# ACCtools/alignasm

Measured on AMD Instinct MI355X. Metric: contigs_per_sec, higher is better.
Workload: dtype int64

## Files before the change

alignasm_amd/csrc/aasm_kernels.h:

```cpp
#pragma once
#include <cstddef>
#include "aasm_dev.h"
#include "../../include/alignasm_amd.h"

namespace aasm {

struct PqK;
struct WS {
    int64_t C, R, R0, S, VT, ET;
    int32_t K, nsl;
    int32_t avg_sidetracks;
    int32_t xcd_map;
    int32_t mw_compact;
    int32_t sort_depth_test;
    const int64_t *rec_off, *in_qs, *in_qe, *in_rs, *in_re, *in_qt, *in_rng_off, *rql, *rqr, *rrl;
    const int32_t *in_chr;
    const uint8_t *in_fwd, *in_mq;
    const char *cs_text;
    const int64_t *cs_off;
    int64_t *rng_rec;
    int64_t rng_stride;
    int32_t *cs_bad;
    int32_t *perm, *dupflag, *np, *pstart;
    int64_t *s_qs, *s_qe, *s_rs, *s_re, *s_qt, *s_rb;
    int32_t *s_rn, *s_chr, *s_orig, *s_ctg, *s_pid;
    uint8_t *s_fl;
    int32_t *ov_cnt, *ov_rec, *ov_vid;
    int64_t *ov_off, *ov_rank, *ov_peq, *ov_per, *ov_stq, *ov_str;
    uint8_t *ov_ok;
    int32_t *dis_end, *next_cnt;
    int32_t *ctgV, *v_i, *v_j, *v_ctg;
    int64_t *voff, *v_slot;
    int32_t *deg, *e_col, *e_wr, *indeg, *rcur, *r_e;
    I4 *tmp_pk;
    int64_t *rowptr, *e_wq, *rptr;
    uint8_t *e_fl;
    Dist *sp_d;
    int32_t *sp_best, *rev_order, *cnt_tmp, *fwd_order, *fwd_pos, *an, *anom_dest, *cnt_tmp2;
    int32_t *tp_deg, *tp_vj;
    int64_t *tp_ptr;
    I4 *te_pk;
    int32_t *ccnt, *cval;
    int64_t *hoff;
    int32_t *hcap_cnt;
    HNode *hnodes;
    int32_t *h_root, *bq, *h_cnt;
    Dist *kd;
    int32_t *klast, *kfound;
    I4 *kcand;
    PqK *pq;
    int64_t pq_stride;
    int32_t *pathA, *pathB, *pathT, *pre2, *stamp;
    Dist *dist2;
    uint8_t *notalt;
    int32_t *mark_time;
    int32_t *plan_kk;
    int32_t *nconv, *cv_ctg, *cv_k, *cv_ord, *cv_kind, *cv_szr, *cv_szv, *cv_n, *cv_err, *cv_path, *cv_pre2, *cv_stamp, *cv_la;
    int64_t *conv_off, *cv_roff, *cv_voff, *cv_cov;
    OutElem *cv_out;
    Dist *cv_dist2;
    int64_t NCONV;
    OutElem *cur_out, *main_out, *alt_out, *pool;
    int32_t *main_len, *alt_len, *all_gen, *all_seq;
    int32_t *ar_ctg, *ar_gen, *ar_seq, *ar_len;
    int64_t *ar_off;
    int64_t pool_cap, ar_cap;
    int64_t *main_off, *alt_off;
    OutElem *main_c, *alt_c;
    int32_t *status;
    int64_t *counters;
    int32_t *gb_flag; int32_t gb_off;
    int64_t *prof_heap, *prof_sel, *prof_gb;
    Dist *st_cost;
    int32_t *st_n;
    I4 *vhdr, *vhdr2, *cinfo;
    int32_t mw_mode;
    int32_t *mw_flag, *mw_lg;
    HNode *hprov;
    int64_t *mw_off;
    int32_t *mw_cap;
    int32_t *mw_order, *mw_rs, *mw_fb;
    int32_t *mw_rsv, *mw_used;
    int32_t *mw_list, *mw_sorted;
    int32_t *mw_key;
    int32_t mw_n, mw_base;
    I4 *tnx;
    int32_t *tnx16;
    I4 *rvh;
    I4 *r_pk;
    I4 *fvh;
    int32_t chain_mode;
    int32_t chain_all, chain_minN;
    int32_t chain_test;
    int32_t *chain_flag, *chain_list;
    int32_t *pend;
    int32_t *cq;
    I4 *bfsq;
    int32_t chain_ord;
    int32_t chain_rn;
};

enum { CNT_RANGE_STEPS = 0, CNT_UNCONN, CNT_POOL, CNT_AR, CNT_CONVERTED, CNT_HEAPNODES, CNT_PATHS, CNT_OVF, CNT_ISPR_E, CNT_ISPR_V, CNT_PATH_E, CNT_OUT_E, CNT_PQ_PUSH, CNT_MW, CNT_MAXN, CNT_LONGSORT, CNT_MAXV, CNT_CHAIN, CNT_GB_S, CNT_GB_L, CNT_GB_REST, CNT_N };

AASM_DEV void set_status(const WS &w, int64_t c, int code) { if (w.status[c] == 0) w.status[c] = code; }
AASM_DEV bool in_chain_class(const WS &w, int64_t c) { return w.chain_flag != nullptr && w.chain_flag[c] != 0; }
AASM_DEV bool in_graph_class(const WS &w, int64_t c) { return w.gb_flag && w.gb_flag[c] != 0; }
#define AASM_COORD_LIMIT ((int64_t)1 << 40)
AASM_DEV bool coord_ok(int64_t x) { return x >= 0 && x < AASM_COORD_LIMIT; }

AASM_DEV bool cs_is_op(int c) { return c == ':' || c == '*' || c == '+' || c == '-'; }
struct CsScan {
    int64_t q, rr, val, n, cnt, o0;
    int32_t plen;
    int t;
    bool fwd, bad;
};
AASM_DEV void cs_close_op(CsScan &s, const WS &w) {
    if (s.t == ':') {
        if (s.plen < 1 || s.val <= 0 || s.n >= s.cnt) { s.bad = true; return; }
        if (s.fwd) {
            const int64_t o = s.o0 + s.n;
            I4 lo, hi; const int64_t qr = s.q + s.val - 1;
            lo.x = lo32((uint64_t)s.q); lo.y = hi32((uint64_t)s.q); lo.z = lo32((uint64_t)qr); lo.w = hi32((uint64_t)qr);
            hi.x = lo32((uint64_t)s.rr); hi.y = hi32((uint64_t)s.rr); hi.z = 0; hi.w = 0;
            I4 *rec = (I4 *)(w.rng_rec + 4 * o); rec[0] = lo; rec[1] = hi;
            s.q += s.val;
        } else {
            const int64_t o = s.o0 + s.cnt - 1 - s.n;
            I4 lo, hi; const int64_t ql = s.q - s.val, qr = s.q - 1, rl = s.rr + s.val - 1;
            lo.x = lo32((uint64_t)ql); lo.y = hi32((uint64_t)ql); lo.z = lo32((uint64_t)qr); lo.w = hi32((uint64_t)qr);
            hi.x = lo32((uint64_t)rl); hi.y = hi32((uint64_t)rl); hi.z = 0; hi.w = 0;
            I4 *rec = (I4 *)(w.rng_rec + 4 * o); rec[0] = lo; rec[1] = hi;
            s.q -= s.val;
        }
        s.rr += s.val;
        s.n++;
    } else if (s.t == '*') {
        if (s.plen != 2) { s.bad = true; return; }
        s.q += s.fwd ? 1 : -1; s.rr += 1;
    } else {
        if (s.plen < 1) { s.bad = true; return; }
        if (s.t == '+') s.q += s.fwd ? s.plen : -s.plen; else s.rr += s.plen;
    }
}
AASM_DEV void kb_cs_ranges(const KCtx &k, const WS &w) {
    const int64_t br = k.bid * k.nthreads + k.tid;
    if (br >= w.R) return;
    const int64_t r = w.R0 + br;
    const int64_t p0 = w.cs_off[r], len = w.cs_off[r + 1] - p0;
    const uint8_t *cs = (const uint8_t *)w.cs_text + p0;
    const int64_t qs = w.in_qs[r], qe = w.in_qe[r], rs = w.in_rs[r], re = w.in_re[r];
    CsScan s;
    s.fwd = w.in_fwd[r] != 0;
    s.o0 = w.in_rng_off[r]; s.cnt = w.in_rng_off[r + 1] - s.o0;
    s.q = s.fwd ? qs : qe + 1; s.rr = s.fwd ? rs : re;
// ... 1818 lines not shown
    if (gv >= w.VT || in_chain_class(w, w.v_ctg[gv]) || in_graph_class(w, w.v_ctg[gv])) return;
    tnx16_vertex(w, gv);
}
#define TNX_TPB 256
#define AASM_TNXWG_LDS_BYTES (GB_MAXV_L * 4)
AASM_DEV void kb_tnx16_wg(const KCtx &k, const WS &w) {
    const int64_t c = k.bid;
    const int64_t V = w.ctgV[c];
    if (V == 0 || !in_graph_class(w, c) || in_chain_class(w, c)) return;
    int32_t *Lb = (int32_t *)k.lds;
    const int64_t vb = w.voff[c];
    for (int32_t v = k.tid; v < V; v += k.nthreads) Lb[v] = w.sp_best[vb + v];
    block_barrier();
    for (int32_t v = k.tid; v < V; v += k.nthreads) {
        I4 *o = (I4 *)(w.tnx16 + 16 * (vb + v));
        int32_t x = v;
        AASM_UNROLL
        for (int t = 0; t < 4; t++) {
            I4 j;
            x = x >= 0 ? Lb[x] : -1; j.x = x;
            x = x >= 0 ? Lb[x] : -1; j.y = x;
            x = x >= 0 ? Lb[x] : -1; j.z = x;
            x = x >= 0 ? Lb[x] : -1; j.w = x;
            o[t] = j;
        }
    }
}
AASM_DEV void kb_k7_prep(const KCtx &k, const WS &w) {
    const int64_t gv = k.bid * k.nthreads + k.tid;
    if (gv >= w.VT || in_chain_class(w, w.v_ctg[gv])) return;
    int32_t ch4[4];
    const int32_t nch = children_vertex(w, gv, ch4);
    const int32_t nkeys = sidetrack_vertex(w, gv);
    I4 a, b;
    heap_hdr_vertex(w, gv, a, b, nch, ch4, nkeys);
    w.vhdr[gv] = a; w.vhdr2[gv] = b;
}
AASM_DEV void kb_heap_hdr(const KCtx &k, const WS &w) {
    const int64_t gv = k.bid * k.nthreads + k.tid;
    if (gv >= w.VT || in_chain_class(w, w.v_ctg[gv])) return;
    I4 a, b;
    heap_hdr_vertex(w, gv, a, b);
    w.vhdr[gv] = a; w.vhdr2[gv] = b;
}

AASM_DEV void kb_heap_cap(const KCtx &k, const WS &w) {
    const int64_t c = k.bid * k.nthreads + k.tid;
    if (c >= w.C) return;
    const int64_t V = w.ctgV[c];
    w.mw_flag[c] = 0; w.mw_cap[c] = 0; w.mw_lg[c] = 2;
    if (w.chain_flag) w.chain_flag[c] = 0;
    w.gb_flag[c] = 0;
    if (V == 0) { w.hcap_cnt[c] = 0; return; }
    const int64_t vb = w.voff[c];
    const int64_t E = w.rowptr[vb + V] - w.rowptr[vb];
    {
        const bool sparse_batch = w.rowptr[w.VT] <= 6 * w.VT;
        const int32_t f = (w.gb_off || !sparse_batch) ? 0 : (V <= GB_MAXV && E <= GB_MAXE) ? 1 : (V <= GB_MAXV_L && E <= GB_MAXE_L) ? 2 : 0;
        w.gb_flag[c] = f;
        atomic_add(&w.counters[f == 1 ? CNT_GB_S : f == 2 ? CNT_GB_L : CNT_GB_REST], (int64_t)1);
    }
    if (E > (int64_t)INT32_MAX - 64) { w.status[c] = -5; w.hcap_cnt[c] = 0; return; }
    int64_t I = E - (V - 1);
    if (I < 0) I = 0;
    int lg = 0;
    for (int64_t t = I + 1; t > 1; t >>= 1) lg++;
    int64_t cap = I * (lg + 2) + 8;
    if (cap > 0x7fffff00) cap = 0x7fffff00;
    w.mw_lg[c] = lg + 2;
    w.mw_flag[c] = (w.mw_mode == 1 || (w.mw_mode == 0 && I >= 6 * V && V >= 128)) ? 1 : 0;
    w.mw_cap[c] = w.mw_flag[c] ? (int32_t)cap : 0;
    w.hcap_cnt[c] = (w.mw_flag[c] && !w.mw_compact) ? 0 : (int32_t)cap;
    if (w.mw_flag[c]) { const int64_t slot = atomic_add(&w.counters[CNT_MW], (int64_t)1); w.mw_list[slot] = (int32_t)c; w.mw_key[slot] = (int32_t)cap; }
    if (w.chain_flag) {
        const int64_t N = w.rec_off[c + 1] - w.rec_off[c];
        const bool sparse_batch = w.rowptr[w.VT] <= 6 * w.VT;
        const bool in = !w.mw_flag[c] && sparse_batch && w.status[c] == 0 &&
                        (w.chain_mode == 1 || (w.chain_mode == 0 && (w.chain_all || (w.chain_minN > 0 && N >= w.chain_minN))));
        w.chain_flag[c] = in ? 1 : 0;
        if (in) { const int64_t slot = atomic_add(&w.counters[CNT_CHAIN], (int64_t)1); w.chain_list[slot] = (int32_t)c; }
    }
}

#define HEAP_RING 64
#define HEAP_QN 128
#define HEAP_KMAX 16
struct HeapStage { Dist key[HEAP_KMAX]; };
#define HEAP_OLDN 8
template <int RING, int QN> struct HeapLdsT {
    HNode ring[RING];
    I4 bq[QN];
    HeapStage stage;
    HNode bounce;
    HNode oldn[HEAP_OLDN];
};
#define HEAP_RING_1W 64
#define HEAP_QN_1W 128
#define HEAP_RING_CH 256
#define HEAP_QN_CH 128
#define AASM_HEAP_LDS_BYTES_T(RING, QN) ((RING) * 48 + (QN) * 16 + HEAP_KMAX * 32 + 48 + HEAP_OLDN * 48)
#define AASM_HEAP_LDS_BYTES AASM_HEAP_LDS_BYTES_T(HEAP_RING_1W, HEAP_QN_1W)
static_assert(sizeof(HeapLdsT<HEAP_RING_1W, HEAP_QN_1W>) <= AASM_HEAP_LDS_BYTES && sizeof(HeapLdsT<HEAP_RING_CH, HEAP_QN_CH>) <= AASM_HEAP_LDS_BYTES_T(HEAP_RING_CH, HEAP_QN_CH), "LDS budget");
struct Spine {
    LaneArr<NodeQ> n;
    LaneArr<int32_t> idx;
    LaneArr<int64_t> sum;
    LaneArr<int32_t> t;
    int32_t root, len, tail;
};
struct HeapState {
    HNode *nodes;
    HNode *ring;
    int32_t rn;
    HNode *bounce;
    HNode *oldn;
    int32_t alloc, flushed, cap;
    int32_t ring_lo;
    bool ovf;
};

AASM_DEV const HNode *heap_arena(const WS &w, int64_t c) { return (w.mw_flag[c] && !w.mw_compact) ? w.hprov + w.mw_off[c] : w.hnodes + w.hoff[c]; }
AASM_DEV NodeQ heap_read(const HeapState &hs, int32_t a, HNode *slot = nullptr) {
    NodeQ n;
    const HNode *src = &hs.ring[a & (hs.rn - 1)];
    if (!slot) slot = hs.bounce;
    if (!(a >= hs.alloc - hs.rn && a >= hs.ring_lo)) {
        const NodeQ g = nodeq_load(&hs.nodes[a]);
        asm volatile("" ::: "memory");
        nodeq_store(slot, g);
        src = slot;
    }
    n = nodeq_load(src);
    return n;
}
AASM_DEV bool nodeq_key_lt(const NodeQ &n, const Dist &key, int64_t ksum) {
    const Dist nk = nodeq_key(n);
    const int64_t nsum = nk.qry + nk.ref;
    if (nsum != ksum && nsum != -2 && ksum != -2) return nsum < ksum;
    return dist_lt<CALC_SUM_MODE>(nk, key);
}
AASM_DEV bool key_tie_lt(const NodeQ &n, const Dist &key) {
    const int32_t na = n.q1.x, nn = n.q1.y, nt = n.q1.z ? n.q1.z : 1, kt = key.qtot ? key.qtot : 1;
    return (na < key.anom) | ((na == key.anom) & ((int64_t)nn * (int64_t)kt > (int64_t)key.qnz * (int64_t)nt));
}
AASM_DEV void heap_flush(HeapState &hs, int lane) {
    const int32_t m = hs.alloc - hs.flushed;
    if (m > 0) {
        wave_lds_sync();
        FOR_LANE(t, m, lane) { const int32_t a = hs.flushed + t; nodeq_store(&hs.nodes[a], nodeq_load(&hs.ring[a & (hs.rn - 1)])); }
        hs.flushed = hs.alloc;
    }
}

template <bool UNI_CHASE, class KP>
AASM_DEV int32_t heap_insert(HeapState &hs, Spine &sp, int32_t hu, const Dist key, int32_t eu, int32_t ev, int lane, KP &kp) {
    const int64_t ksum = key.qry + key.ref;
    if (hu != sp.root) { sp.root = hu; sp.len = 0; sp.tail = hu; }
    int32_t depth = -1, a_stop = -1, a_rank = 0;
    if (sp.len > 0) {
        uint64_t lt = wave_index_mask(sp.len, lane, [&](int j) { return sp.sum.at(j) < ksum; });
        const uint64_t eq = wave_index_mask(sp.len, lane, [&](int j) { return sp.sum.at(j) == ksum; });
        if (eq) lt |= wave_index_mask(sp.len, lane, [&](int j) { return sp.sum.at(j) == ksum && key_tie_lt(sp.n.at(j), key); });
        const uint64_t stop = ~lt & lanemask_lt(sp.len);
        if (stop) { depth = ffs64(stop) - 1; a_stop = LA_GET(sp.idx, depth, ); a_rank = LA_GET(sp.n, depth, .q1.w) & 0xff; }
    }
    if (depth < 0 && UNI_CHASE) {
        depth = sp.len;
        int32_t a = sp.tail;
        const int32_t d0 = depth;
        int32_t my_a = -1, my_slot = -1;
        int32_t nold = 0;
        if (a >= 0) wave_lds_sync();
        while (a >= 0) {
            if (depth >= AASM_WAVE_MAX - 2) { hs.ovf = true; return -1; }
            const bool in_ring = a >= hs.alloc - hs.rn && a >= hs.ring_lo;
#if defined(AASM_HOST_EMUL)
            const NodeQ n = heap_read(hs, a);
#else
            const NodeQ n = heap_read(hs, a, (!in_ring && nold < HEAP_OLDN) ? &hs.oldn[nold] : nullptr);
#endif
#if defined(AASM_KPROF) && !defined(AASM_HOST_EMUL)
            if (lane == 0) kp.acc[in_ring ? 7 : 6] += 1;
#endif
            const int64_t nsum = nodeq_key(n).qry + nodeq_key(n).ref;
#if defined(AASM_HOST_EMUL)
            FOR_LANE_EQ(j, depth, lane) { sp.n.at(j) = n; sp.idx.at(j) = a; sp.sum.at(j) = nsum; }
            (void)in_ring; (void)nold; (void)my_slot;
#else
            if (lane == depth) { my_a = a; my_slot = in_ring ? -1 : (nold < HEAP_OLDN ? nold : -2); }
            if (!in_ring) nold++;
#endif
            bool lt = wave_any(nsum < ksum);
            if (!lt && wave_any(nsum == ksum)) lt = wave_any(key_tie_lt(n, key));
            if (!lt) { a_rank = uni(n.q1.w) & 0xff; break; }
            a = uni(n.q2.y);
            depth++;
        }
        a_stop = a;
#if defined(AASM_HOST_EMUL)
        (void)d0; (void)my_a;
#else
        if (depth > d0 && my_a >= 0) {
            const HNode *src = my_slot >= 0 ? &hs.oldn[my_slot] : &hs.ring[my_a & (hs.rn - 1)];
            NodeQ n = nodeq_load(src);
            if (my_slot == -2) { n = nodeq_load(&hs.nodes[my_a]); asm volatile("" ::: "memory"); }
            sp.n.r = n; sp.idx.r = my_a; sp.sum.r = nodeq_key(n).qry + nodeq_key(n).ref;
        }
#endif
    }
    if (depth < 0 && !UNI_CHASE) {
        depth = sp.len;
        int32_t a = sp.tail;
        if (a >= 0) wave_lds_sync();
        while (a >= 0) {
            if (depth >= AASM_WAVE_MAX - 2) { hs.ovf = true; return -1; }
            bool lt = false;
            FOR_LANE_EQ(j, depth, lane) {
                const NodeQ n = heap_read(hs, a);
#if defined(AASM_KPROF) && !defined(AASM_HOST_EMUL)
                kp.acc[(a >= hs.alloc - hs.rn && a >= hs.ring_lo) ? 7 : 6] += 1;
#endif
                const int64_t nsum = nodeq_key(n).qry + nodeq_key(n).ref;
                sp.n.at(j) = n; sp.idx.at(j) = a; sp.sum.at(j) = nsum;
                lt = (nsum < ksum) | ((nsum == ksum) & key_tie_lt(n, key));
            }
            if (!wave_ballot(lt)) { a_rank = LA_GET(sp.n, depth, .q1.w) & 0xff; break; }
            a = LA_GET(sp.n, depth, .q2.y);
            depth++;
        }
        a_stop = a;
    }
    if (hs.alloc + depth + 1 > hs.cap) { hs.ovf = true; return -1; }
    if (hs.alloc + depth + 1 - hs.flushed > HEAP_RING) heap_flush(hs, lane);
    FOR_LANE(j, depth + 1, lane) {
        const NodeQ &nj = sp.n.at(j);
        const int32_t aj = (nj.q2.x < 0) ? 0 : (((nj.q1.w >> 8) & 0xff) + 1);
        sp.t.at(j) = ((j == depth) ? 1 : aj) + j;
    }
    lane_excl_suffix_min(sp.t, depth + 1, lane);
    const int32_t alloc = hs.alloc, nalloc = alloc + depth + 1;
    uint64_t swm = 0;
#if defined(AASM_HOST_EMUL)
    for (int j = 0; j <= depth; j++)
#else
    const int j = lane;
    const bool in = j <= depth;
#endif
    {
        const bool leaf = (j == depth);
        const NodeQ old = sp.n.at(j);
        const int32_t l = old.q2.x, l_rank = (old.q1.w >> 8) & 0xff, r_rank = sp.t.at(j) - (j + 1);
        const bool sw = (l < 0) | (l_rank < r_rank);
        const bool has_right = sw ? (l >= 0) : true;
        const int32_t nr_rank = has_right ? (sw ? l_rank : r_rank) : 0;
        const int32_t nrank = has_right ? nr_rank + 1 : 0;
        const int32_t ni = alloc + (depth - j), below = ni - 1;
        NodeQ n;
        n.q0.x = leaf ? (int32_t)(uint32_t)(uint64_t)key.qry : old.q0.x; n.q0.y = leaf ? (int32_t)((uint64_t)key.qry >> 32) : old.q0.y;
        n.q0.z = leaf ? (int32_t)(uint32_t)(uint64_t)key.ref : old.q0.z; n.q0.w = leaf ? (int32_t)((uint64_t)key.ref >> 32) : old.q0.w;
        n.q1.x = leaf ? key.anom : old.q1.x; n.q1.y = leaf ? key.qnz : old.q1.y; n.q1.z = leaf ? key.qtot : old.q1.z;
        n.q1.w = leaf ? (1 | (a_rank << 8)) : (nrank | ((sw ? r_rank : l_rank) << 8) | (nr_rank << 16));
        n.q2.x = leaf ? a_stop : (sw ? below : l); n.q2.y = leaf ? -1 : (sw ? l : below);
        n.q2.z = leaf ? eu : old.q2.z; n.q2.w = leaf ? ev : old.q2.w;
#if defined(AASM_HOST_EMUL)
        nodeq_store(&hs.ring[ni & (hs.rn - 1)], n);
        sp.n.at(j) = n; sp.idx.at(j) = ni; if (leaf) sp.sum.at(j) = ksum;
        if (!leaf && sw) swm |= 1ull << j;
#else
        if (in) {
            nodeq_store(&hs.ring[ni & (hs.rn - 1)], n);
            sp.n.at(j) = n; sp.idx.at(j) = ni; if (leaf) sp.sum.at(j) = ksum;
        }
        swm = wave_ballot(in && !leaf && sw);
#endif
    }
    if (swm) { const int t = ffs64(swm) - 1; sp.len = t + 1; sp.tail = LA_GET(sp.n, t, .q2.y); }
    else { sp.len = depth + 1; sp.tail = -1; }
    sp.root = alloc + depth;
    hs.alloc = nalloc;
    return sp.root;
}

struct KProfNone { int64_t acc[8]; };
AASM_DEV bool chain_wait_hdr(ChainSync *S, const I4 *vh, const I4 *vh2, int32_t u, int64_t patience) {
    const int64_t t0 = wave_realtime();
    int64_t guard = 0;
    for (;;) {
        const int32_t pd = uni(ld_shared_i32(&S->prep_done));
        const int32_t x = uni(ld_shared_i32(&vh[u].x)), y = uni(ld_shared_i32(&vh2[u].y));
        if (x != -1 && y != -1) { wave_fence(); return true; }
        if (pd) return false;
        if ((++guard & 1023) == 0 && wave_realtime() - t0 > patience) return false;
        wave_sleep();
    }
}
template <bool CHAIN = false, int RING = HEAP_RING_1W, int QN = HEAP_QN_1W>
AASM_DEV void kb_heap(const KCtx &k, const WS &w, ChainSync *S = nullptr) {
    const int64_t c = k.bid;
    const int64_t V = w.ctgV[c];
    if (V == 0) return;
    if (!CHAIN && in_chain_class(w, c)) return;
    HeapLdsT<RING, QN> *L = (HeapLdsT<RING, QN> *)k.lds;
    const int64_t vb = w.voff[c];
    int32_t *h = w.h_root + vb, *q = w.bq + vb;
    const I4 *vh = w.vhdr + vb, *vh2 = w.vhdr2 + vb;
    const Dist *sk = w.st_cost + w.rowptr[vb];
    HeapState hs;
    hs.nodes = w.hnodes + w.hoff[c]; hs.ring = L->ring; hs.rn = RING; hs.bounce = &L->bounce; hs.oldn = L->oldn; hs.alloc = 0; hs.flushed = 0; hs.ring_lo = 0; hs.ovf = false;
    hs.cap = (int32_t)(w.hoff[c + 1] - w.hoff[c]);
    const int32_t src = (int32_t)(V - 2), dest = (int32_t)(V - 1);
    if (w.mw_flag[c]) return;
#if !defined(AASM_HOST_EMUL)
    {
        const int64_t I = (w.rowptr[vb + V] - w.rowptr[vb]) - (V - 1);
        const int64_t a = w.avg_sidetracks > 0 ? w.avg_sidetracks : 1;
        if (8 * I > 9 * a) __builtin_amdgcn_s_setprio(3);
        else if (I > a) __builtin_amdgcn_s_setprio(2);
        else if (8 * I > 7 * a) __builtin_amdgcn_s_setprio(1);
    }
#endif
    if (k.lane == 0) w.h_cnt[c] = 0;
    if (w.status[c] != 0) return;
    if (!CHAIN && dist_is_max(w.sp_d[vb + src])) { if (k.lane == 0) set_status(w, c, -6); return; }
    bool chain_lost = false;
    const int64_t patience = (CHAIN && w.chain_test == 2) ? (int64_t)100000000 : (int64_t)30 * 100000000;
    int32_t head = 0, tail = 0, lds_hi = 0;
    Spine sp; sp.root = -2; sp.len = 0; sp.tail = -1;
#if defined(AASM_KPROF) && !defined(AASM_HOST_EMUL)
    KPROF_DECL;
    KPROF_START();
    struct KP { int64_t &t0; int64_t *acc; } kp{kp_t0, kp_acc};
#else
    KProfNone kp;
#endif
    int32_t u = dest, hu = -1, so = 0, n = 0;
    if (CHAIN && !chain_wait_hdr(S, vh, vh2, dest, patience)) chain_lost = true;
    else {
        const I4 a0 = vh[dest];
        so = uni(a0.x); n = uni(a0.y);
    }
    wave_lds_sync();
    int32_t pend_u = -1, pend_root = -1;
    int32_t staged = -1;
    int32_t c_nch = 0, c_fc = -1, c_sofc = 0, c_nfc = 0, c_c0lo = 0, c_c0hi = 0, c_n = 0;
    while (!hs.ovf && !chain_lost) {
        HeapStage *St = &L->stage;
        if (staged != u) {
            if (CHAIN && !chain_wait_hdr(S, vh, vh2, u, patience)) { chain_lost = true; break; }
            const I4 ha = vh[u], hb = vh2[u];
            so = uni(ha.x); c_n = uni(ha.y);
            FOR_LANE(t, (c_n < HEAP_KMAX ? c_n : HEAP_KMAX), k.lane) { const Dist kk = sk[(int64_t)so + t]; St->key[t] = kk; }
            c_nch = uni(ha.z); c_fc = uni(ha.w); c_sofc = uni(hb.z); c_nfc = uni(hb.w); c_c0lo = uni(hb.x); c_c0hi = uni(hb.y);
            wave_lds_sync();
        }
        n = c_n;
        const int32_t nch = c_nch, fc = c_fc, so_fc = c_sofc, n_fc = c_nfc, c0lo = c_c0lo, c0hi = c_c0hi;
        KPROF_STAMP(0);
        if (pend_u >= 0) h[pend_u] = pend_root;
        if (hs.alloc - hs.flushed >= HEAP_RING / 2) heap_flush(hs, k.lane);
        KPROF_STAMP(1);
        int32_t v2 = -1, so2 = 0, n2 = 0, hu2 = -1;
        bool peeked = false;
        if (head < tail) { if (head < lds_hi) { const I4 e = L->bq[head & (QN - 1)]; v2 = uni(e.x); hu2 = uni(e.y); so2 = uni(e.z); n2 = uni(e.w); peeked = true; } }
        else if (nch > 0) { v2 = fc; so2 = so_fc; n2 = n_fc; }
        I4 pa, pb;
        LaneArr<Dist> pk;
        pa.x = pa.y = pa.z = pa.w = 0; pb = pa;
#if !defined(AASM_HOST_EMUL)
        pk.r = dist_zero();
#endif
        if (v2 >= 0) {
            pa = vh[v2]; pb = vh2[v2];
            FOR_LANE(t, (n2 < HEAP_KMAX ? n2 : HEAP_KMAX), k.lane) pk.at(t) = sk[(int64_t)so2 + t];
        }
        I4 cpre;
        cpre.x = cpre.y = cpre.z = cpre.w = 0;
        const int64_t c0 = (int64_t)(((uint64_t)(uint32_t)c0hi << 32) | (uint32_t)c0lo);
        if (nch > 0 && !(nch == 1 && head == tail) && k.lane < nch) cpre = w.cinfo[c0 + k.lane];
        KPROF_STAMP(2);
        for (int32_t t = 0; t < n && !hs.ovf; t++) {
            if (t >= HEAP_KMAX && (t & (HEAP_KMAX - 1)) == 0) {
                wave_lds_sync();
                FOR_LANE(j, (n - t < HEAP_KMAX ? n - t : HEAP_KMAX), k.lane) { const Dist kk = sk[(int64_t)so + t + j]; St->key[j] = kk; }
                wave_lds_sync();
            }
            const Dist cc = St->key[t & (HEAP_KMAX - 1)];
            hu = heap_insert<true>(hs, sp, hu, cc, u, cc.pad, k.lane, kp);
        }
        KPROF_STAMP(3);
        pend_u = (k.lane == 0) ? u : -1; pend_root = hu;
        bool v2_ok = v2 >= 0;
        if (CHAIN && v2_ok && (uni(pa.x) == -1 || uni(pb.y) == -1)) v2_ok = false;
        if (v2_ok) {
            c_nch = uni(pa.z); c_fc = uni(pa.w); c_sofc = uni(pb.z); c_nfc = uni(pb.w); c_c0lo = uni(pb.x); c_c0hi = uni(pb.y); c_n = uni(pa.y);
            FOR_LANE(t, (n2 < HEAP_KMAX ? n2 : HEAP_KMAX), k.lane) St->key[t] = pk.at(t);
        }
        staged = v2_ok ? v2 : -1;
        if (nch == 1 && head == tail) {
            u = fc; so = so_fc; n = n_fc;
            wave_lds_sync();
            continue;
        }
        if (nch > 0) {
            int32_t ncache = 0;
            if (lds_hi == tail) { ncache = QN - (tail - head); if (ncache > nch) ncache = nch; if (ncache < 0) ncache = 0; }
            for (int32_t t = k.lane; t < nch; t += AASM_WAVE) {
                I4 ci = cpre;
                if (t >= AASM_WAVE) ci = w.cinfo[c0 + t];
                if (t < ncache) { I4 e; e.x = ci.x; e.y = hu; e.z = ci.y; e.w = ci.z; L->bq[(tail + t) & (QN - 1)] = e; }
                else { h[ci.x] = hu; q[tail + t] = ci.x; }
            }
            lds_hi += ncache;
            tail += nch;
        }
        wave_lds_sync();
        KPROF_STAMP(4);
        if (head >= tail) break;
        if (peeked) { u = v2; hu = hu2; so = so2; n = n2; }
        else if (head < lds_hi) { const I4 e = L->bq[head & (QN - 1)]; u = uni(e.x); hu = uni(e.y); so = uni(e.z); n = uni(e.w); }
        else {
            wave_fence();
            u = uni(q[head]); hu = uni(h[u]);
            const I4 a0 = vh[u]; so = uni(a0.x); n = uni(a0.y);
        }
        head++;
        if (head >= lds_hi && head == tail) lds_hi = tail;
        KPROF_STAMP(5);
    }
    if (pend_u >= 0) h[pend_u] = pend_root;
    heap_flush(hs, k.lane);
    KPROF_FLUSH(w.prof_heap, c, k.lane);
    if (CHAIN) {
        const int64_t t0 = wave_realtime();
        int64_t guard = 0;
        while (!chain_lost && !uni(ld_shared_i32(&S->sweep_done))) {
            if ((++guard & 1023) == 0 && wave_realtime() - t0 > patience) chain_lost = true;
            wave_sleep();
        }
        wave_fence();
        if (chain_lost || uni(ld_shared_i32(&w.sp_d[vb + src].anom)) < 0) { if (k.lane == 0) { set_status(w, c, -6); w.h_cnt[c] = 0; } return; }
    }
    if (hs.ovf) { if (k.lane == 0) set_status(w, c, -5); return; }
    if (k.lane == 0) { w.h_cnt[c] = hs.alloc; atomic_add(&w.counters[CNT_HEAPNODES], (int64_t)hs.alloc); }
}

#define AASM_CHAIN_LDS_BYTES (AASM_REV_LDS_BYTES + AASM_HEAP_LDS_BYTES_T(HEAP_RING_CH, HEAP_QN_CH) + 32)
#define CHAIN_WAVES 4
#define CHAIN_LONG_ROW 8
struct ChainLds { RevQ rq; HeapLdsT<HEAP_RING_CH, HEAP_QN_CH> hl; ChainSync s; };
static_assert(sizeof(ChainLds) <= AASM_CHAIN_LDS_BYTES, "LDS budget");

AASM_DEV void chain_prep(const KCtx &k, const WS &w, int64_t c, ChainSync *S) {
    const int64_t vb = w.voff[c];
    const int32_t *q = w.rev_order + vb;
    int32_t *pend = w.pend + vb, *cq = w.cq + vb;
    int32_t done1 = 0, r2_head = 0, r2_tail = 0;
    const int64_t t_start = wave_realtime();
    int64_t guard = 0;
    int32_t result = 1;
    for (;;) {
        const int32_t sd = uni(ld_shared_i32(&S->sweep_done));
        const int32_t t = uni(ld_shared_i32(&S->tail_pub));
        wave_fence();
        bool did = false;
        if (done1 < t) {
            const int32_t n1 = (t - done1 < AASM_WAVE) ? (t - done1) : AASM_WAVE;
            int32_t v = -1, deg = 0;
            int64_t r0 = 0;
            bool self = false;
            if (k.lane < n1) {
                v = q[done1 + k.lane];
                sidetrack_vertex(w, vb + v);
                tnx_vertex(w, vb + v);
                r0 = w.rowptr[vb + v]; deg = (int32_t)(w.rowptr[vb + v + 1] - r0);
                self = w.rptr[vb + v + 1] == w.rptr[vb + v];
            }
            wave_fence();
            {
                const uint64_t m = wave_ballot(self);
                if (self) cq[r2_tail + popc64(m & lanemask_lt(k.lane))] = v;
                r2_tail += popc64(m);
            }
            const bool longrow = deg > CHAIN_LONG_ROW;
            for (int32_t e = 0; wave_any(!longrow && e < deg); e++) {
                bool hit = false;
                int32_t x = -1;
                if (!longrow && e < deg) { x = w.e_col[r0 + e]; hit = atomic_add(&pend[x], (int32_t)-1) == 1; }
                const uint64_t m = wave_ballot(hit);
                if (hit) cq[r2_tail + popc64(m & lanemask_lt(k.lane))] = x;
                r2_tail += popc64(m);
            }
            uint64_t lm = wave_ballot(longrow);
            while (lm) {
                const int sl = ffs64(lm) - 1;
                lm &= lm - 1;
                const int64_t r02 = wave_bcast(r0, sl);
                const int32_t deg2 = wave_bcast(deg, sl);
                for (int32_t e0 = 0; e0 < deg2; e0 += AASM_WAVE) {
                    const int32_t e = e0 + k.lane;
                    bool hit = false;
                    int32_t x = -1;
                    if (e < deg2) { x = w.e_col[r02 + e]; hit = atomic_add(&pend[x], (int32_t)-1) == 1; }
                    const uint64_t m = wave_ballot(hit);
                    if (hit) cq[r2_tail + popc64(m & lanemask_lt(k.lane))] = x;
                    r2_tail += popc64(m);
                }
            }
            done1 += n1;
            did = true;
            wave_fence();
        }
        if (r2_head < r2_tail) {
            const int32_t n2 = (r2_tail - r2_head < AASM_WAVE) ? (r2_tail - r2_head) : AASM_WAVE;
            int32_t u = -1, nch = 0, ch4[4] = {-1, -1, -1, -1};
            if (k.lane < n2) { u = cq[r2_head + k.lane]; nch = children_vertex(w, vb + u, ch4); }
            wave_fence();
            I4 a, b;
            a.x = a.y = a.z = a.w = 0; b = a;
            if (k.lane < n2) { heap_hdr_vertex(w, vb + u, a, b, nch, ch4, -1); tnx16_vertex(w, vb + u); }
            wave_fence();
            if (k.lane < n2 && !(w.chain_test && c == 0 && u == (int32_t)w.ctgV[c] - 1)) { w.vhdr2[vb + u] = b; w.vhdr[vb + u] = a; }
            r2_head += n2;
            did = true;
            wave_fence();
        }
        if (!did) {
            if (sd && done1 >= t && r2_head == r2_tail) break;
            if ((++guard & 1023) == 0 && wave_realtime() - t_start > (int64_t)60 * 100000000) { result = 2; break; }
            wave_sleep();
        }
    }
    store_drain();
    if (!(w.chain_test == 2 && c == 0)) st_shared_i32(&S->prep_done, result);
}

AASM_DEV void chain_order(const KCtx &k, const WS &w, int64_t c, ChainSync *S) {
    const int64_t V = w.ctgV[c], vb = w.voff[c];
    int32_t result = 1;
    if (V > 0 && w.status[c] == 0 && !w.mw_flag[c]) {
        I4 *q = w.bfsq + vb;
        const I4 *vh = w.vhdr + vb, *vh2 = w.vhdr2 + vb;
        const int64_t patience = (w.chain_test == 2) ? (int64_t)100000000 : (int64_t)30 * 100000000;
        int32_t head = 0, tail = 1;
        if (k.lane == 0) { I4 r; r.x = (int32_t)(V - 1); r.y = -1; r.z = 0; r.w = 0; q[0] = r; }
        wave_fence();
        while (head < tail) {
            const int32_t nb = (tail - head < AASM_WAVE) ? (tail - head) : AASM_WAVE;
            I4 rec; rec.x = -1; rec.y = -1; rec.z = 0; rec.w = 0;
            bool rdy = false;
            wave_fence();
            if (k.lane < nb) {
                rec = q[head + k.lane];
                rdy = ld_shared_i32(&vh[rec.x].x) != -1 && ld_shared_i32(&vh2[rec.x].y) != -1;
            }
            const uint64_t rm = wave_ballot(rdy);
            int32_t r = (~rm == 0ull) ? AASM_WAVE : ffs64(~rm) - 1;
            if (r == 0) {
                if (!chain_wait_hdr(S, vh, vh2, uni(rec.x), patience)) { result = 2; break; }
                r = 1;
            }
            wave_fence();
            int32_t nch = 0;
            int64_t c0 = 0;
            if (k.lane < r) {
                const I4 ha = vh[rec.x], hb = vh2[rec.x];
                rec.z = ha.x; rec.w = ha.y; nch = ha.z;
                c0 = (int64_t)(((uint64_t)(uint32_t)hb.y << 32) | (uint32_t)hb.x);
            }
            const int32_t incl = wave_incl_add(nch);
            const int32_t tot = wave_bcast(incl, AASM_WAVE - 1);
            if (k.lane < r) {
                q[head + k.lane] = rec;
                int32_t at = tail + incl - nch;
                for (int32_t t = 0; t < nch; t++) {
                    const I4 ci = w.cinfo[c0 + t];
                    I4 ch; ch.x = ci.x; ch.y = head + k.lane; ch.z = ci.y; ch.w = 0;
                    q[at + t] = ch;
                }
            }
            head += r; tail += tot;
            store_drain();
            st_shared_i32(&S->ord_pub, head);
        }
    }
    store_drain();
    st_shared_i32(&S->ord_done, result);
}

template <int RING, int QN>
AASM_DEV void kb_heap_ord(const KCtx &k, const WS &w, ChainSync *S) {
    const int64_t c = k.bid;
    const int64_t V = w.ctgV[c];
    if (V == 0) return;
    HeapLdsT<RING, QN> *L = (HeapLdsT<RING, QN> *)k.lds;
    const int64_t vb = w.voff[c];
    int32_t *h = w.h_root + vb;
    const Dist *sk = w.st_cost + w.rowptr[vb];
    const I4 *q = w.bfsq + vb;
    int32_t *rroot = (int32_t *)L->bq;
    const int32_t RN = w.chain_rn > 0 ? w.chain_rn : QN * 4;
    HeapState hs;
    hs.nodes = w.hnodes + w.hoff[c]; hs.ring = L->ring; hs.rn = RING; hs.bounce = &L->bounce; hs.oldn = L->oldn; hs.alloc = 0; hs.flushed = 0; hs.ring_lo = 0; hs.ovf = false;
    hs.cap = (int32_t)(w.hoff[c + 1] - w.hoff[c]);
    const int32_t src = (int32_t)(V - 2);
    if (w.mw_flag[c]) return;
    if (k.lane == 0) w.h_cnt[c] = 0;
    if (w.status[c] != 0) return;
    bool lost = false;
    const int64_t patience = (w.chain_test == 2) ? (int64_t)100000000 : (int64_t)30 * 100000000;
    Spine sp; sp.root = -2; sp.len = 0; sp.tail = -1;
    KProfNone kp;
    HeapStage *St = &L->stage;
    int32_t i = 0;
    int32_t u = -1, p = -1, so = 0, n = 0;
    bool have = false;
    int32_t a_u = -1, a_p = -1, a_so = 0, a_n = 0;
    bool a_have = false;
    int32_t pend_u = -1, pend_root = -1;
    int32_t pub = 0;
    while (!hs.ovf) {
        if (!have) {
            const int64_t t0 = wave_realtime();
            int64_t guard = 0;
            bool end = false;
            for (;;) {
                const int32_t od = uni(ld_shared_i32(&S->ord_done));
                pub = uni(ld_shared_i32(&S->ord_pub));
                if (i < pub) break;
                if (od) { end = true; lost = od == 2; break; }
                if ((++guard & 1023) == 0 && wave_realtime() - t0 > patience) { end = true; lost = true; break; }
                wave_sleep();
            }
            if (end) break;
            wave_fence();
            const I4 r0 = q[i];
            u = uni(r0.x); p = uni(r0.y); so = uni(r0.z); n = uni(r0.w);
            wave_lds_sync();
            FOR_LANE(t, (n < HEAP_KMAX ? n : HEAP_KMAX), k.lane) { const Dist kk = sk[(int64_t)so + t]; St->key[t] = kk; }
            wave_lds_sync();
            have = true; a_have = false;
        }
        int32_t hu = -1;
        if (p >= 0) {
            if (i - p <= RN) hu = uni(rroot[p & (RN - 1)]);
            else { wave_fence(); hu = uni(h[uni(q[p].x)]); }
        }
        if (pend_u >= 0) h[pend_u] = pend_root;
        if (hs.alloc - hs.flushed >= HEAP_RING / 2) heap_flush(hs, k.lane);
        pub = uni(ld_shared_i32(&S->ord_pub));
        if (!a_have && i + 1 < pub) {
            wave_fence();
            const I4 r1 = q[i + 1];
            a_u = uni(r1.x); a_p = uni(r1.y); a_so = uni(r1.z); a_n = uni(r1.w);
            a_have = true;
        }
        LaneArr<Dist> pk;
        I4 rb;
        rb.x = rb.y = rb.z = rb.w = 0;
#if !defined(AASM_HOST_EMUL)
        pk.r = dist_zero();
#endif
        const bool b_have = a_have && i + 2 < pub;
        if (a_have) { FOR_LANE(t, (a_n < HEAP_KMAX ? a_n : HEAP_KMAX), k.lane) pk.at(t) = sk[(int64_t)a_so + t]; }
        if (b_have) rb = q[i + 2];
        for (int32_t t = 0; t < n && !hs.ovf; t++) {
            if (t >= HEAP_KMAX && (t & (HEAP_KMAX - 1)) == 0) {
                wave_lds_sync();
                FOR_LANE(j, (n - t < HEAP_KMAX ? n - t : HEAP_KMAX), k.lane) { const Dist kk = sk[(int64_t)so + t + j]; St->key[j] = kk; }
                wave_lds_sync();
            }
            const Dist cc = St->key[t & (HEAP_KMAX - 1)];
            hu = heap_insert<true>(hs, sp, hu, cc, u, cc.pad, k.lane, kp);
        }
        pend_u = (k.lane == 0) ? u : -1; pend_root = hu;
        wave_lds_sync();
        if (k.lane == 0) rroot[i & (RN - 1)] = hu;
        if (a_have) { FOR_LANE(t, (a_n < HEAP_KMAX ? a_n : HEAP_KMAX), k.lane) St->key[t] = pk.at(t); }
        wave_lds_sync();
        have = a_have; u = a_u; p = a_p; so = a_so; n = a_n;
        a_have = b_have;
        if (b_have) { a_u = uni(rb.x); a_p = uni(rb.y); a_so = uni(rb.z); a_n = uni(rb.w); }
        i++;
    }
    if (pend_u >= 0) h[pend_u] = pend_root;
    heap_flush(hs, k.lane);
    {
        const int64_t t0 = wave_realtime();
        int64_t guard = 0;
        while (!lost && !uni(ld_shared_i32(&S->sweep_done))) {
            if ((++guard & 1023) == 0 && wave_realtime() - t0 > patience) lost = true;
            wave_sleep();
        }
        wave_fence();
        if (lost || uni(ld_shared_i32(&w.sp_d[vb + src].anom)) < 0) { if (k.lane == 0) { set_status(w, c, -6); w.h_cnt[c] = 0; } return; }
    }
    if (hs.ovf) { if (k.lane == 0) set_status(w, c, -5); return; }
    if (k.lane == 0) { w.h_cnt[c] = hs.alloc; atomic_add(&w.counters[CNT_HEAPNODES], (int64_t)hs.alloc); }
}

#if defined(AASM_HOST_EMUL)
AASM_DEV const WS &chain_role_ws(const WS &w) { return w; }
#else
AASM_DEV const WS &chain_role_ws(const WS &) {
    const WS *p = (const WS *)__builtin_amdgcn_kernarg_segment_ptr();
    asm volatile("" : "+s"(p));
    return *p;
}
#endif
template <bool ORD>
AASM_DEV void kb_chain(const KCtx &k, const WS &w) {
    ChainLds *L = (ChainLds *)k.lds;
    const int64_t c = w.chain_list[k.bid];
    const int wv = k.tid / AASM_WAVE;
    if (k.tid == 0) { L->s.tail_pub = 0; L->s.sweep_done = 0; L->s.prep_done = 0; L->s.ord_pub = 0; L->s.ord_done = 0; }
    block_barrier();
    KCtx k2 = k;
    k2.bid = c; k2.tid = k.lane; k2.nthreads = AASM_WAVE;
    if (wv == 0) {
        k2.lds = (char *)&L->rq;
        kb_rev_sweep<AASM_WAVE, true>(k2, chain_role_ws(w), &L->s);
    } else if (wv == 1) {
        chain_prep(k2, chain_role_ws(w), c, &L->s);
    } else if (wv == 2) {
        if (ORD) chain_order(k2, chain_role_ws(w), c, &L->s);
        else {
#if !defined(AASM_HOST_EMUL)
            __builtin_amdgcn_s_setprio(1);
#endif
            k2.lds = (char *)&L->hl;
            kb_heap<true, HEAP_RING_CH, HEAP_QN_CH>(k2, w, &L->s);
        }
    } else if (ORD) {
#if !defined(AASM_HOST_EMUL)
        __builtin_amdgcn_s_setprio(1);
#endif
        k2.lds = (char *)&L->hl;
        kb_heap_ord<HEAP_RING_CH, HEAP_QN_CH>(k2, w, &L->s);
    }
}

#define MW_WAVES 16
struct MwLds {
    int32_t q_head, q_tail, n_done, n_total, stop, n_nodes, pad0, pad1;
    HNode bounce[MW_WAVES];
    HNode ring[MW_WAVES][HEAP_RING];
};
#define AASM_MW_LDS_BYTES(waves) ((waves) * HEAP_RING * 48 + 32 + MW_WAVES * 48)
static_assert(sizeof(MwLds) <= AASM_MW_LDS_BYTES(MW_WAVES), "LDS budget");

AASM_DEV int32_t mw_last_le(const int32_t *a, int32_t n, int32_t x) {
    int32_t lo = 0, hi = n;
    while (hi - lo > 1) { const int32_t m = (lo + hi) >> 1; if (a[m] <= x) lo = m; else hi = m; }
    return lo;
}

AASM_DEV void kb_mw_rank(const KCtx &k, const WS &w) {
    const int64_t i = k.bid * k.nthreads + k.tid;
    if (i >= w.mw_n) return;
    const int32_t ci = w.mw_list[i], key = w.mw_key[i];
    int32_t r = 0;
    int64_t j = 0;
    for (; j + 8 <= w.mw_n; j += 8) {
        int32_t kj[8], cj[8];
        AASM_UNROLL
        for (int u = 0; u < 8; u++) { kj[u] = w.mw_key[j + u]; cj[u] = w.mw_list[j + u]; }
        AASM_UNROLL
        for (int u = 0; u < 8; u++) r += (kj[u] > key || (kj[u] == key && cj[u] < ci)) ? 1 : 0;
    }
    for (; j < w.mw_n; j++) { const int32_t kj = w.mw_key[j], cj = w.mw_list[j]; r += (kj > key || (kj == key && cj < ci)) ? 1 : 0; }
    w.mw_sorted[r] = ci;
}

AASM_DEV void kb_heap_mw(const KCtx &k, const WS &w) {
    const int64_t c = (w.mw_base >= 0) ? (int64_t)w.mw_sorted[w.mw_base + k.bid] : k.bid;
    const int64_t V = w.ctgV[c];
    if (V == 0 || !w.mw_flag[c]) return;
    MwLds *L = (MwLds *)k.lds;
    const int64_t vb = w.voff[c];
    const int wv = k.tid / AASM_WAVE;
    int32_t *h = w.h_root + vb, *q = w.bq + vb;
    const I4 *vh = w.vhdr + vb, *vh2 = w.vhdr2 + vb;
    const Dist *sk = w.st_cost + w.rowptr[vb];
    int32_t *order = w.mw_order + vb, *rs = w.mw_rs + vb, *fb = w.mw_fb + vb, *rsv = w.mw_rsv + vb, *used = w.mw_used + vb;
    const int32_t src = (int32_t)(V - 2), dest = (int32_t)(V - 1);
    const int32_t per_insert = w.mw_lg[c];
    if (k.tid == 0) w.h_cnt[c] = 0;
    if (w.status[c] != 0) return;
    if (dist_is_max(w.sp_d[vb + src])) { if (k.tid == 0) set_status(w, c, -6); return; }
#if defined(AASM_KPROF) && !defined(AASM_HOST_EMUL)
    const int64_t mwp_t0 = wave_realtime();
    int64_t mwp_t1 = 0, mwp_t2 = 0, mwp_t3 = 0;
#define MWP_STAMP(x) do { x = wave_realtime(); } while (0)
#else
#define MWP_STAMP(x) do {} while (0)
#endif
    if (wv == 0) {
        if (k.lane == 0) order[0] = dest;
        wave_fence();
        int32_t n = 1, head = 0, rbase = 0;
        while (head < n) {
            const int32_t chunk = (n - head < AASM_WAVE) ? (n - head) : AASM_WAVE;
            int32_t v = -1, nch = 0, nin = 0;
            int64_t c0 = 0;
            if (k.lane < chunk) {
                v = order[head + k.lane];
                const I4 a = vh[v], b = vh2[v];
                nin = a.y; nch = a.z;
                c0 = (int64_t)(((uint64_t)(uint32_t)b.y << 32) | (uint32_t)b.x);
            }
            const int32_t capv = nin * per_insert, cincl = wave_incl_add(capv), nincl = wave_incl_add(nch);
            if (k.lane < chunk) { rs[head + k.lane] = rbase + cincl - capv; rsv[v] = rbase + cincl - capv; used[v] = 0; }
            for (int32_t j = 0; j < nch; j++) order[n + (nincl - nch) + j] = w.cval[c0 + j];
            rbase += wave_bcast(cincl, AASM_WAVE - 1);
            n += wave_bcast(nincl, AASM_WAVE - 1);
            head += chunk;
            wave_fence();
        }
        if (k.lane == 0) { L->n_total = n; L->q_head = 0; L->q_tail = 0; L->n_done = 0; L->stop = 0; L->n_nodes = 0; }
        store_drain();
    }
    block_barrier();
    MWP_STAMP(mwp_t1);
    const int32_t nv = uni(ld_shared_i32(&L->n_total));
    HeapState hs;
    hs.nodes = w.hprov + w.mw_off[c]; hs.ring = L->ring[wv]; hs.rn = HEAP_RING; hs.bounce = &L->bounce[wv]; hs.oldn = nullptr; hs.alloc = 0; hs.flushed = 0; hs.ring_lo = 0; hs.cap = 0; hs.ovf = false;
// ... 1322 lines not shown
```

Before: 451,500.

## Walk in-ring heap spine with hand-written GCN assembly loop

Adds an inline-assembly loop that follows the heap spine while nodes are still in the LDS ring. It reads each node with ds_read, compares the key with scalar branches, and records the lane index through m0/writelane. Control returns to the C++ path when the walk leaves the ring or hits the depth limit. The aim is to cut the per-node overhead of the generic heap_read/compare path in heap_insert. The cost is hard-coded VGPR clobbers (v40-v48), m0 save and restore, and extra compiler memory barriers at the call sites, all of which can raise register pressure or constrain scheduling.

```diff
diff --git a/alignasm_amd/csrc/aasm_k7_asm.h b/alignasm_amd/csrc/aasm_k7_asm.h
--- /dev/null
+++ b/alignasm_amd/csrc/aasm_k7_asm.h
@@ -0,0 +1,79 @@
+#pragma once
+#include "aasm_dev.h"
+
+#if !defined(AASM_K7_ASM)
+#define AASM_K7_ASM 1
+#endif
+#if !defined(AASM_K7_ASM_CHAIN)
+#define AASM_K7_ASM_CHAIN 1
+#endif
+
+namespace aasm {
+
+enum { K7W_END = 0, K7W_STOP = 1, K7W_CXX = 2 };
+
+#if !defined(AASM_HOST_EMUL)
+AASM_DEV int32_t k7_walk_ring(int32_t &a, int32_t &depth, int32_t &rank, int32_t &my_a, uint32_t ring_lds, int32_t rmask,
+                              int32_t lo, int64_t ksum, int32_t kanom, int32_t kqnz, int32_t kt) {
+    int32_t why, keep, t, va, nt;
+    uint64_t m;
+    int64_t sum, p0, p1;
+    asm volatile(
+        "s_mov_b32 %[keep], m0\n\t"
+        "s_mov_b32 m0, %[d]\n\t"
+        "s_mov_b32 %[why], 0\n"
+        "1:\n\t"
+        "s_cmp_lt_i32 %[a], 0\n\t"
+        "s_cbranch_scc1 5f\n\t"
+        "s_cmp_ge_i32 m0, 62\n\t"
+        "s_cbranch_scc1 4f\n\t"
+        "s_cmp_lt_i32 %[a], %[lo]\n\t"
+        "s_cbranch_scc1 4f\n\t"
+        "s_and_b32 %[t], %[a], %[rmask]\n\t"
+        "s_mul_i32 %[t], %[t], 48\n\t"
+        "s_add_u32 %[t], %[t], %[base]\n\t"
+        "v_mov_b32 %[va], %[t]\n\t"
+        "ds_read_b128 v[40:43], %[va]\n\t"
+        "ds_read_b128 v[44:47], %[va] offset:16\n\t"
+        "ds_read_b32 v48, %[va] offset:36\n\t"
+        "v_writelane_b32 %[mya], %[a], m0\n\t"
+        "s_waitcnt lgkmcnt(0)\n\t"
+        "v_lshl_add_u64 %[sum], v[40:41], 0, v[42:43]\n\t"
+        "v_cmp_lt_i64_e32 vcc, %[sum], %[ksum]\n\t"
+        "s_cbranch_vccnz 2f\n\t"
+        "v_cmp_eq_u64_e32 vcc, %[sum], %[ksum]\n\t"
+        "s_cbranch_vccz 3f\n\t"
+        "v_max_u32_e32 %[nt], 1, v46\n\t"
+        "v_mad_i64_i32 %[p0], %[m], v45, %[kt], 0\n\t"
+        "v_mad_i64_i32 %[p1], %[m], %[kqnz], %[nt], 0\n\t"
+        "v_cmp_gt_i64_e32 vcc, %[p0], %[p1]\n\t"
+        "v_cmp_eq_u32_e64 %[m], v44, %[kanom]\n\t"
+        "s_and_b64 vcc, vcc, %[m]\n\t"
+        "v_cmp_lt_i32_e64 %[m], v44, %[kanom]\n\t"
+        "s_or_b64 %[m], vcc, %[m]\n\t"
+        "s_cbranch_scc0 3f\n"
+        "2:\n\t"
+        "v_readfirstlane_b32 %[a], v48\n\t"
+        "s_add_u32 m0, m0, 1\n\t"
+        "s_branch 1b\n"
+        "3:\n\t"
+        "v_readfirstlane_b32 %[rank], v47\n\t"
+        "s_and_b32 %[rank], %[rank], 0xff\n\t"
+        "s_mov_b32 %[why], 1\n\t"
+        "s_branch 5f\n"
+        "4:\n\t"
+        "s_mov_b32 %[why], 2\n"
+        "5:\n\t"
+        "s_mov_b32 %[d], m0\n\t"
+        "s_mov_b32 m0, %[keep]\n\t"
+        "s_nop 4"
+        : [a] "+s"(a), [d] "+s"(depth), [rank] "+s"(rank), [mya] "+v"(my_a), [why] "=&s"(why), [keep] "=&s"(keep),
+          [t] "=&s"(t), [m] "=&s"(m), [va] "=&v"(va), [nt] "=&v"(nt), [sum] "=&v"(sum), [p0] "=&v"(p0), [p1] "=&v"(p1)
+        : [base] "s"(ring_lds), [rmask] "s"(rmask), [lo] "s"(lo), [ksum] "v"(ksum), [kanom] "v"(kanom), [kqnz] "v"(kqnz),
+          [kt] "v"(kt)
+        : "vcc", "scc", "memory", "v40", "v41", "v42", "v43", "v44", "v45", "v46", "v47", "v48");
+    return why;
+}
+#endif
+
+}
diff --git a/alignasm_amd/csrc/aasm_kernels.h b/alignasm_amd/csrc/aasm_kernels.h
--- a/alignasm_amd/csrc/aasm_kernels.h
+++ b/alignasm_amd/csrc/aasm_kernels.h
@@ -1,6 +1,7 @@
 #pragma once
 #include <cstddef>
 #include "aasm_dev.h"
+#include "aasm_k7_asm.h"
 #include "../../include/alignasm_amd.h"
 
 namespace aasm {
@@ -2125,7 +2126,7 @@
     }
 }
 
-template <bool UNI_CHASE, class KP>
+template <bool UNI_CHASE, bool WALK_ASM = false, class KP>
 AASM_DEV int32_t heap_insert(HeapState &hs, Spine &sp, int32_t hu, const Dist key, int32_t eu, int32_t ev, int lane, KP &kp) {
     const int64_t ksum = key.qry + key.ref;
     if (hu != sp.root) { sp.root = hu; sp.len = 0; sp.tail = hu; }
@@ -2144,7 +2145,24 @@
         int32_t my_a = -1, my_slot = -1;
         int32_t nold = 0;
         if (a >= 0) wave_lds_sync();
+#if !defined(AASM_HOST_EMUL)
+        const int32_t ring_min = uni(hs.ring_lo > hs.alloc - hs.rn ? hs.ring_lo : hs.alloc - hs.rn);
+        const int32_t key_t = key.qtot ? key.qtot : 1;
+#endif
         while (a >= 0) {
+#if !defined(AASM_HOST_EMUL)
+            if (WALK_ASM && AASM_K7_ASM) {
+                const int32_t d_in = depth;
+                const int32_t why = k7_walk_ring(a, depth, a_rank, my_a, (uint32_t)(uintptr_t)hs.ring, uni(hs.rn - 1), ring_min, ksum,
+                                                 key.anom, key.qnz, key_t);
+#if defined(AASM_KPROF)
+                if (lane == 0) kp.acc[7] += depth - d_in + (why == K7W_STOP);
+#else
+                (void)d_in;
+#endif
+                if (why != K7W_CXX) break;
+            }
+#endif
             if (depth >= AASM_WAVE_MAX - 2) { hs.ovf = true; return -1; }
             const bool in_ring = a >= hs.alloc - hs.rn && a >= hs.ring_lo;
 #if defined(AASM_HOST_EMUL)
@@ -2344,6 +2362,7 @@
 #endif
         if (v2 >= 0) {
             pa = vh[v2]; pb = vh2[v2];
+            if (CHAIN) asm volatile("" ::: "memory");
             FOR_LANE(t, (n2 < HEAP_KMAX ? n2 : HEAP_KMAX), k.lane) pk.at(t) = sk[(int64_t)so2 + t];
         }
         I4 cpre;
@@ -2358,7 +2377,7 @@
                 wave_lds_sync();
             }
             const Dist cc = St->key[t & (HEAP_KMAX - 1)];
-            hu = heap_insert<true>(hs, sp, hu, cc, u, cc.pad, k.lane, kp);
+            hu = heap_insert<true, (CHAIN ? AASM_K7_ASM_CHAIN : AASM_K7_ASM) != 0>(hs, sp, hu, cc, u, cc.pad, k.lane, kp);
         }
         KPROF_STAMP(3);
         pend_u = (k.lane == 0) ? u : -1; pend_root = hu;
@@ -2621,6 +2640,7 @@
         if (pend_u >= 0) h[pend_u] = pend_root;
         if (hs.alloc - hs.flushed >= HEAP_RING / 2) heap_flush(hs, k.lane);
         pub = uni(ld_shared_i32(&S->ord_pub));
+        asm volatile("" ::: "memory");
         if (!a_have && i + 1 < pub) {
             wave_fence();
             const I4 r1 = q[i + 1];
@@ -2643,7 +2663,7 @@
                 wave_lds_sync();
             }
             const Dist cc = St->key[t & (HEAP_KMAX - 1)];
-            hu = heap_insert<true>(hs, sp, hu, cc, u, cc.pad, k.lane, kp);
+            hu = heap_insert<true, AASM_K7_ASM_CHAIN != 0>(hs, sp, hu, cc, u, cc.pad, k.lane, kp);
         }
         pend_u = (k.lane == 0) ? u : -1; pend_root = hu;
         wave_lds_sync();
```

Result: no change. 451,800, median of 6 (+0.1%).
